# zdebruine/singlet

Measured on AMD Instinct MI355X. Metric: ALS iterations/sec (1M cells x 30k genes, 5% nnz, k=50), higher is better.
Workload: dtype f64

## Files before the change

### singlet_amd/csrc/kernels_tiled.hip

```cpp
#include "sgl_internal.h"
#include <atomic>
#include <hipcub/hipcub.hpp>
#include <stdlib.h>
#include <utility>
#include <type_traits>

#define TILED_NW 8
#define TILED_CW 64
#define TILED_NP 32
#define TILED_LDS_BYTES (160 * 1024 - 512)
#define TILED_SLACK 4096

__device__ __forceinline__ int64_t tiled_slot_col(const int32_t* __restrict__ perm, int64_t ncol, int64_t wb, int h, int p, int nsl) {
    const int64_t pos = wb * (TILED_NP * nsl) + nsl * p + h;
    if (pos >= ncol) return -1;
    return perm ? (int64_t)perm[pos] : pos;
}

__device__ __forceinline__ int tiled_ranges_of(int64_t wb, int R, int64_t tail_wg0, int tail_R) {
    return (tail_R > 1 && tail_wg0 >= 0 && wb / TILED_NW >= tail_wg0) ? tail_R : R;
}
__device__ __forceinline__ int tiled_range_end(int b, int T, int NB, int nr) {
    const int t = b >> 1;
    const int y = (int)(((int64_t)(t + 1) * nr - 1) / T);
    const int b1 = 2 * (int)(((int64_t)(y + 1) * T) / nr);
    return b1 < NB ? b1 : NB;
}

__global__ __launch_bounds__(256) void tiled_count_kernel(const int64_t* __restrict__ seg, const int32_t* __restrict__ perm, int64_t ncol,
                                                          int T, int NB, int64_t nwb, int R, int64_t tail_wg0, int tail_R,
                                                          uint8_t* __restrict__ cnt, uint16_t* __restrict__ ahead,
                                                          int64_t* __restrict__ chunk_entries, int nsl) {
    const int lane = threadIdx.x & 63, p = lane & 31;
    const int64_t wb = ((int64_t)blockIdx.x * blockDim.x + threadIdx.x) >> 6;
    if (wb >= nwb) return;
    const int gps = 16 / nsl;
    int64_t col[4];
    for (int h = 0; h < 4; ++h) col[h] = h < nsl ? tiled_slot_col(perm, ncol, wb, h, p, nsl) : -1;
    const int nr = tiled_ranges_of(wb, R, tail_wg0, tail_R);
    for (int b0 = 0; b0 < NB;) {
        const int b1 = tiled_range_end(b0, T, NB, nr);
        int64_t pos[4];
        for (int h = 0; h < 4; ++h) pos[h] = col[h] >= 0 ? seg[(int64_t)b0 * ncol + col[h]] : 0;
        for (int b = b0; b < b1; ++b) {
            const int hi = b + 2 < b1 ? b + 2 : b1;
            int64_t must = 0, avail = 0, ew[4];
            for (int h = 0; h < 4; ++h) {
                ew[h] = 0;
                if (col[h] >= 0) {
                    const int64_t eb = seg[(int64_t)(b + 1) * ncol + col[h]];
                    ew[h] = seg[(int64_t)hi * ncol + col[h]];
                    must = eb - pos[h] > must ? eb - pos[h] : must;
                    avail = ew[h] - pos[h] > avail ? ew[h] - pos[h] : avail;
                }
            }
            int g = (int)((must + 3) >> 2);
            const int cap = (int)((avail + 3) >> 2) - g;
            int tot = g;
            for (int o = 16; o > 0; o >>= 1) tot += __shfl_xor(tot, o, 32);
            const int rem = (gps - (tot & (gps - 1))) & (gps - 1);
            int suf = cap;
            for (int o = 1; o < 32; o <<= 1) {
                const int v = __shfl_down(suf, o, 32);
                if (p + o < 32) suf += v;
            }
            const int above = suf - cap;
            int extra = rem - above < cap ? rem - above : cap;
            if (extra < 0) extra = 0;
            const int all = __shfl(suf, 0, 32);
            if (p == TILED_NP - 1 && rem > all) extra += rem - all;
            g += extra;
            const int64_t u = wb * NB + b;
            if (lane < 32) {
                cnt[u * TILED_NP + p] = (uint8_t)g;
                for (int h = 0; h < nsl; ++h)
                    ahead[u * (TILED_NP * nsl) + nsl * p + h] = col[h] >= 0 ? (uint16_t)(pos[h] - seg[(int64_t)b * ncol + col[h]]) : (uint16_t)0;
            }
            if (lane == 0) chunk_entries[u] = (int64_t)(tot + rem) * 4 * nsl;
            for (int h = 0; h < 4; ++h) pos[h] += (4 * (int64_t)g < ew[h] - pos[h]) ? 4 * (int64_t)g : ew[h] - pos[h];
        }
        b0 = b1;
    }
}

__global__ __launch_bounds__(256) void tiled_fill_kernel(const double* __restrict__ x, const int32_t* __restrict__ idx,
                                                         const int64_t* __restrict__ seg, const int32_t* __restrict__ perm,
                                                         int64_t ncol, int T, int NB, int64_t nwb, int R, int64_t tail_wg0, int tail_R,
                                                         int D, int row_bytes, const uint8_t* __restrict__ cnt,
                                                         const uint16_t* __restrict__ ahead, const int64_t* __restrict__ cstart,
                                                         uint32_t* __restrict__ sroff, double* __restrict__ sx,
                                                         int masked, uint64_t seed, SglDiv inv_density, int mask_t,
                                                         int64_t col_off, int64_t row_off, int nsl) {
    const int lane = threadIdx.x & 63;
    const int eps = 64 / nsl, eps_sh = nsl == 4 ? 4 : 5;
    const int64_t gw = ((int64_t)blockIdx.x * blockDim.x + threadIdx.x) >> 6;
    const int64_t nw = ((int64_t)gridDim.x * blockDim.x) >> 6;
    for (int64_t u = gw; u < nwb * NB; u += nw) {
        const int64_t wb = u / NB;
        const int b = (int)(u - wb * NB);
        const int b1 = tiled_range_end(b, T, NB, tiled_ranges_of(wb, R, tail_wg0, tail_R));
        const int hi = b + 2 < b1 ? b + 2 : b1;
        const int64_t c0 = cstart[u];
        int P = 0;
        for (int p = 0; p < TILED_NP; ++p) {
            const int n4 = 4 * (int)cnt[u * TILED_NP + p];
            if (n4 == 0) continue;
            for (int h = 0; h < nsl; ++h) {
                const int64_t col = tiled_slot_col(perm, ncol, wb, h, p, nsl);
                int64_t a = 0, e = 0;
                if (col >= 0) {
                    a = seg[(int64_t)b * ncol + col] + ahead[u * (TILED_NP * nsl) + nsl * p + h];
                    e = seg[(int64_t)hi * ncol + col];
                }
                for (int q = lane; q < n4; q += 64) {
                    uint32_t ro = 0;
                    double xv = 0.0;
                    if (a + q < e) {
                        const int32_t r = idx[a + q];
                        const int blk = r >= (b + 1) * D ? b + 1 : b;
                        ro = (uint32_t)((blk & 1) * D + (r - blk * D)) * (uint32_t)row_bytes;
                        xv = x[a + q];
                        if (masked) {
                            const uint64_t gc = (uint64_t)(col + col_off), gr = (uint64_t)(r + row_off);
                            if (mask_t ? sgl_draw(seed, gr, gc, inv_density) : sgl_draw(seed, gc, gr, inv_density)) xv = 0.0;
                        }
                    }
                    const int pos = P + q;
                    const int64_t dst = c0 + (int64_t)(pos >> eps_sh) * 64 + h * eps + (pos & (eps - 1));
                    if (sroff != nullptr) sroff[dst] = ro;
                    sx[dst] = xv;
                }
            }
            P += n4;
        }
    }
}

__global__ __launch_bounds__(256) void tiled_gtab_kernel(const uint8_t* __restrict__ cnt, const int64_t* __restrict__ cstart,
                                                         int64_t nchunks, int nsl, uint16_t* __restrict__ gtab) {
    const int lane = threadIdx.x & 63;
    const int64_t gw = ((int64_t)blockIdx.x * blockDim.x + threadIdx.x) >> 6;
    const int64_t nw = ((int64_t)gridDim.x * blockDim.x) >> 6;
    for (int64_t u = gw; u < nchunks; u += nw) {
        int64_t g0 = cstart[u] / (4 * nsl);
        for (int p = 0; p < TILED_NP; ++p) {
            const int n = (int)cnt[u * TILED_NP + p];
            for (int q = lane; q < n; q += 64) gtab[g0 + q] = (uint16_t)(0x8000u | (unsigned)(4 * p));
            g0 += n;
        }
    }
}

template <typename T_>
static int t_alloc(T_** p, size_t count) {
    *p = nullptr;
    if (count == 0) count = 1;
    hipError_t e = sgl_pool_malloc((void**)p, count * sizeof(T_));
    if (e != hipSuccess) {
        (void)hipGetLastError();
        sgl_set_error("hipMalloc of %zu bytes failed: %s", count * sizeof(T_), hipGetErrorString(e));
        return SGL_ENOMEM;
    }
    return SGL_OK;
}

template <typename T_>
static int t_reserve(T_** p, size_t* cap, size_t count) {
    if (*p != nullptr && *cap >= count) return SGL_OK;
    if (*p) (void)sgl_pool_free(*p);
    *p = nullptr;
    *cap = 0;
    const size_t want = count + count / 32 + 64;
    SGLCHK(t_alloc(p, want));
    *cap = want;
    return SGL_OK;
}

void sgl_tiled_free(DevTiled& S) {
    if (S.seg) (void)sgl_pool_free(S.seg);
    if (S.perm) (void)sgl_pool_free(S.perm);
    if (S.roff) (void)sgl_pool_free(S.roff);
    if (S.x) (void)sgl_pool_free(S.x);
    if (S.cstart) (void)sgl_pool_free(S.cstart);
    if (S.cnt) (void)sgl_pool_free(S.cnt);
    if (S.ahead) (void)sgl_pool_free(S.ahead);
    if (S.gtab) (void)sgl_pool_free(S.gtab);
    if (S.part) (void)sgl_pool_free(S.part);
    if (S.xm) (void)sgl_pool_free(S.xm);
    S = DevTiled();
}

static bool tiled_sort_columns() {
    const char* e = getenv("SGL_TILED_SORT");
    return !(e && *e == '0');
}

__global__ void tiled_col_keys_kernel(const int64_t* __restrict__ p, int64_t ncol, uint32_t* __restrict__ keys, int32_t* __restrict__ iota) {
    for (int64_t c = (int64_t)blockIdx.x * blockDim.x + threadIdx.x; c < ncol; c += (int64_t)gridDim.x * blockDim.x) {
        keys[c] = (uint32_t)(p[c + 1] - p[c]);
        iota[c] = (int32_t)c;
    }
}

static int tiled_build_perm(sgl_ctx* c, const DevCSC& M, DevTiled& S) {
    hipStream_t s = c->stream;
    const int64_t n = M.ncol;
    SGLCHK(t_reserve(&S.perm, &S.cap_perm, (size_t)n));
    uint32_t *keys = nullptr, *keys_out = nullptr;
    int32_t* iota = nullptr;
    void* tmp = nullptr;
    int rc = t_alloc(&keys, (size_t)n);
    if (rc == SGL_OK) rc = t_alloc(&keys_out, (size_t)n);
    if (rc == SGL_OK) rc = t_alloc(&iota, (size_t)n);
    if (rc == SGL_OK && n > 0) {
        const int64_t blocks = std::min<int64_t>((n + 255) / 256, 4096);
        tiled_col_keys_kernel<<<dim3((unsigned)blocks), dim3(256), 0, s>>>(M.p, n, keys, iota);
        size_t tmp_bytes = 0;
        if (hipcub::DeviceRadixSort::SortPairsDescending(nullptr, tmp_bytes, keys, keys_out, iota, S.perm, n, 0, 32, s) != hipSuccess) rc = SGL_EHIP;
        if (rc == SGL_OK && sgl_pool_malloc(&tmp, tmp_bytes ? tmp_bytes : 1) != hipSuccess) { (void)hipGetLastError(); rc = SGL_ENOMEM; }
        if (rc == SGL_OK && hipcub::DeviceRadixSort::SortPairsDescending(tmp, tmp_bytes, keys, keys_out, iota, S.perm, n, 0, 32, s) != hipSuccess) rc = SGL_EHIP;
    }
    static_assert(TILED_CW == 64, "pair layout: 64 columns per wave");
    std::vector<uint32_t> top_v((size_t)TILED_NW * TILED_CW * 2);
    uint32_t* top = top_v.data();
    const int64_t ntop = std::min<int64_t>(n, (int64_t)top_v.size());
    if (rc == SGL_OK && ntop > 0 && hipMemcpyAsync(top, keys_out, sizeof(uint32_t) * (size_t)ntop, hipMemcpyDeviceToHost, s) != hipSuccess) rc = SGL_EHIP;
    const hipError_t e = hipStreamSynchronize(s);
    if (rc == SGL_OK && e == hipSuccess) {
        int64_t tn = 0, tn2 = 0;
        for (int64_t q = 0; q < ntop; ++q) {
            if (q < TILED_NW * TILED_CW) tn += top[q];
            tn2 += top[q];
        }
        S.top_share = M.nnz > 0 ? (double)tn / (double)M.nnz : 0.0;
        S.top_share4 = M.nnz > 0 ? (double)tn2 / (double)M.nnz : 0.0;
    }
    if (keys) (void)sgl_pool_free(keys);
    if (keys_out) (void)sgl_pool_free(keys_out);
    if (iota) (void)sgl_pool_free(iota);
    if (tmp) (void)sgl_pool_free(tmp);
    if (rc == SGL_OK && e != hipSuccess) rc = SGL_EHIP;
    if (rc != SGL_OK) { sgl_set_error("tiled build: sorting the columns by their non-zero count failed"); return rc; }
    S.perm_nnz = M.nnz;
    return SGL_OK;
}

void sgl_trace_setup(const char* what);

int sgl_tiled_build(sgl_ctx* c, const DevCSC& M, int k, DevTiled& S) {
    hipStream_t s = c->stream;
    const int nsl = (k <= 32 && !getenv("SGL_TILED_NO_QUAD")) ? 4 : 2;
    if (S.built && S.k == k && S.NSL == nsl && S.ncol == M.ncol && S.nrow == M.nrow && S.src_nnz == M.nnz && (S.perm != nullptr) == tiled_sort_columns())
        return SGL_OK;
    S.built = false;
    S.xm_mask_t = -1;
    S.k = k;
    S.NSL = nsl;
    S.CW = TILED_NP * nsl;
    const int KS = nsl == 4 ? 32 : ((k + 1) & ~1);
    S.KS = KS;
    int TR = TILED_LDS_BYTES / (KS * 8);
    TR = TR / 8 * 8;
    if (TR > 984) TR = 984;
    if (TR < 8 || k > 64) { sgl_set_error("tiled accumulate: k=%d unsupported", k); return SGL_EINVAL; }
    S.nwb = ((int64_t)M.ncol + S.CW - 1) / S.CW;
    {
        const int64_t groups = (S.nwb + TILED_NW - 1) / TILED_NW, T0 = ((int64_t)M.nrow + TR - 1) / TR;
        if (groups * T0 < 256 && !getenv("SGL_TILED_FULL_TILES")) {
            const int64_t want = std::min<int64_t>((256 + groups - 1) / groups, ((int64_t)M.nrow + 127) / 128);
            if (want > T0) TR = std::min<int>(TR, (int)(((((int64_t)M.nrow + want - 1) / want) + 7) / 8 * 8));
        }
    }
    S.TR = TR;
    S.T = (int)((M.nrow + TR - 1) / TR);
    const int D = TR / 2;
    S.NB = (int)((M.nrow + D - 1) / D);
    S.ncol = M.ncol;
    S.nrow = M.nrow;
    S.src_nnz = M.nnz;
    const int64_t nchunks = S.nwb * S.NB;

    int rc = SGL_OK;
    if (!tiled_sort_columns()) {
        if (S.perm) { (void)sgl_pool_free(S.perm); S.perm = nullptr; S.cap_perm = 0; }
    } else if (!S.perm || S.perm_nnz != M.nnz || S.cap_perm < (size_t)M.ncol) {
        rc = tiled_build_perm(c, M, S);
    }
    sgl_trace_setup("  stream: column order");
    const double E_est = (double)M.nnz * 1.06;
    const int64_t nwg_x = (S.nwb + TILED_NW - 1) / TILED_NW;
    int R = 1;
    const int r_fill = nwg_x < 1024 ? (int)std::max<int64_t>(1, (512 + nwg_x - 1) / nwg_x) : 1;
    const double top_share = nsl == 4 ? S.top_share4 : S.top_share;
    const bool skewed = S.perm && top_share * (double)nwg_x > 1.5;
    const int r_bal = skewed ? (int)std::min<double>(256.0, ceil(top_share * 256.0 / 0.35)) : 1;
    if (r_bal > r_fill) {
        double best = -1.0;
        const int rmin = std::max(r_fill, (int)std::min<int64_t>(r_bal, std::max(1, S.T)));
        if (rmin > S.T) R = std::max(1, S.T);
        for (int r = rmin; r <= std::min<int64_t>(S.T, rmin + rmin / 4 + 4); ++r) {
            const int tpr = (S.T + r - 1) / r;
            const int reff = (S.T + tpr - 1) / tpr;
            const double wgs = (double)nwg_x * reff;
            const double eff = wgs / (ceil(wgs / 256.0) * 256.0);
            if (eff > best + 1e-9) { best = eff; R = reff; }
        }
    } else if (r_fill > 1 && S.T > 1) {
        const double t_tile = E_est / (double)nsl / ((double)nwg_x * (double)S.T) * 2.4e-9 + 2.5e-6;
        const double t_wg = 6e-6;
        double best = 1e300;
        for (int r = 1; r <= std::min<int64_t>(S.T, 64); ++r) {
            const double wgs = (double)nwg_x * r;
            const double rounds = ceil(wgs / 256.0);
            const int largest = (S.T + r - 1) / r;
            const double cost = rounds * ((double)largest * t_tile + t_wg) + (r > 1 ? (double)r * (double)k * (double)M.ncol * 16.0 / 4e12 : 0.0);
            if (cost < best * (1.0 - 1e-9)) { best = cost; R = r; }
        }
    }
    if (const char* fr = getenv("SGL_TILED_RANGES")) {
        if (atoi(fr) > 0) R = atoi(fr);
    }
    S.range_fastest = r_bal > r_fill;
    S.R = std::max(1, std::min(R, std::max(1, S.T)));
    S.tiles_per_range = (S.T + S.R - 1) / S.R;
    S.tail_wg0 = -1;
    S.tail_R = 1;
    if (S.R == 1 && !S.range_fastest && nwg_x > 256 && S.T > 1 && E_est >= (double)(4ll << 20) && !getenv("SGL_TILED_NO_TAIL")) {
        const int64_t tail = nwg_x % 256;
        if (tail > 0) {
            const double t_tile = E_est / (double)nsl / ((double)nwg_x * (double)S.T) * 2.4e-9 + 2.5e-6;
            const double t_wg = 6e-6;
            const double tail_cols = (double)tail * TILED_NW * S.CW;
            double best = (double)S.T * t_tile + t_wg;
            int Rt = 1;
            for (int r = 2; r <= std::min<int64_t>(S.T, 16); ++r) {
                const double rounds = ceil((double)tail * r / 256.0);
                const double cost = rounds * ((double)((S.T + r - 1) / r) * t_tile + t_wg) + (double)r * (double)k * tail_cols * 16.0 / 4e12;
                if (cost < best * (1.0 - 1e-9)) { best = cost; Rt = r; }
            }
            if (Rt > 1) { S.tail_wg0 = nwg_x - tail; S.tail_R = Rt; }
        }
    }
    if (rc == SGL_OK) rc = t_reserve(&S.seg, &S.cap_seg, (size_t)(S.NB + 1) * (size_t)M.ncol);
    sgl_trace_setup("  stream: segment buffer reserved");
    DevCSC tmp = M;
    tmp.tile_rows = D;
    tmp.ntiles = S.NB;
    tmp.seg = S.seg;
    if (rc == SGL_OK) rc = k_build_segments(s, tmp);
    int64_t* chunk_entries = nullptr;
    if (rc == SGL_OK) rc = t_alloc(&chunk_entries, (size_t)nchunks);
    if (rc == SGL_OK) rc = t_reserve(&S.cnt, &S.cap_cnt, (size_t)nchunks * TILED_NP);
    if (rc == SGL_OK) rc = t_reserve(&S.ahead, &S.cap_ahead, (size_t)nchunks * (size_t)S.CW);
    if (rc == SGL_OK) rc = t_reserve(&S.cstart, &S.cap_cstart, (size_t)nchunks + 1);
    if (rc == SGL_OK && S.nwb > 0) {
        tiled_count_kernel<<<dim3((unsigned)((S.nwb + 3) / 4)), dim3(256), 0, s>>>(S.seg, S.perm, M.ncol, S.T, S.NB, S.nwb, S.R,
                                                                                   S.tail_wg0, S.tail_R, S.cnt, S.ahead, chunk_entries, nsl);
        if (hipGetLastError() != hipSuccess) { sgl_set_error("tiled build: count kernel launch failed"); rc = SGL_EHIP; }
    }
    if (rc == SGL_OK) rc = k_exclusive_scan(c, chunk_entries, S.cstart, nchunks);
    if (rc == SGL_OK) rc = k_scan_total(s, chunk_entries, S.cstart, nchunks);
    int64_t E = 0;
    if (rc == SGL_OK) {
        if (hipMemcpyAsync(&E, S.cstart + nchunks, sizeof(int64_t), hipMemcpyDeviceToHost, s) != hipSuccess ||
            hipStreamSynchronize(s) != hipSuccess) { sgl_set_error("tiled build: reading the stream size failed"); rc = SGL_EHIP; }
    }
    S.E = E;
    sgl_trace_setup("  stream: segments, counts, scan");
    if (rc == SGL_OK) rc = t_reserve(&S.roff, &S.cap_roff, (size_t)E + TILED_SLACK);
    if (rc == SGL_OK) rc = t_reserve(&S.x, &S.cap_x, (size_t)E + TILED_SLACK);
    sgl_trace_setup("  stream: roff / x buffers reserved");
    if (rc == SGL_OK) {
        if (hipMemsetAsync(S.roff + E, 0, TILED_SLACK * sizeof(uint32_t), s) != hipSuccess ||
            hipMemsetAsync(S.x + E, 0, TILED_SLACK * sizeof(double), s) != hipSuccess) { sgl_set_error("tiled build: clearing the stream slack failed"); rc = SGL_EHIP; }
    }
    if (rc == SGL_OK && nchunks > 0) {
        int64_t blocks = (nchunks + 3) / 4;
        if (blocks > 256 * 64) blocks = 256 * 64;
        tiled_fill_kernel<<<dim3((unsigned)blocks), dim3(256), 0, s>>>(M.x, M.i, S.seg, S.perm, M.ncol, S.T, S.NB, S.nwb, S.R, S.tail_wg0,
                                                                       S.tail_R, D, KS * 8, S.cnt, S.ahead, S.cstart, S.roff, S.x,
                                                                       0, 0, sgl_div_make(1), 0, 0, 0, nsl);
        if (hipGetLastError() != hipSuccess) { sgl_set_error("tiled build: fill kernel launch failed"); rc = SGL_EHIP; }
    }
    const size_t ngroups = (size_t)(E / (4 * nsl));
    if (rc == SGL_OK) rc = t_reserve(&S.gtab, &S.cap_gtab, ngroups + 256);
    if (rc == SGL_OK) {
        if (hipMemsetAsync(S.gtab + ngroups, 0, 256 * sizeof(uint16_t), s) != hipSuccess) { sgl_set_error("tiled build: clearing the schedule slack failed"); rc = SGL_EHIP; }
    }
    if (rc == SGL_OK && nchunks > 0) {
        int64_t blocks = (nchunks + 3) / 4;
        if (blocks > 256 * 64) blocks = 256 * 64;
        tiled_gtab_kernel<<<dim3((unsigned)blocks), dim3(256), 0, s>>>(S.cnt, S.cstart, nchunks, nsl, S.gtab);
        if (hipGetLastError() != hipSuccess) { sgl_set_error("tiled build: schedule kernel launch failed"); rc = SGL_EHIP; }
    }
    if (rc == SGL_OK && S.R > 1) rc = t_reserve(&S.part, &S.cap_part, (size_t)S.R * (size_t)k * (size_t)M.ncol);
    if (rc == SGL_OK && S.tail_R > 1)
        rc = t_reserve(&S.part, &S.cap_part, (size_t)S.tail_R * (size_t)k * (size_t)((nwg_x - S.tail_wg0) * TILED_NW * S.CW));
    hipError_t e = hipStreamSynchronize(s);
    if (chunk_entries) (void)sgl_pool_free(chunk_entries);
    if (rc == SGL_OK && e != hipSuccess) { sgl_set_error("tiled build failed: %s", hipGetErrorString(e)); rc = SGL_EHIP; }
    if (rc != SGL_OK) { sgl_tiled_free(S); return rc; }
    S.built = true;
    ++S.builds;
    return rc;
}

int sgl_tiled_mask_values(sgl_ctx* c, const DevCSC& M, DevTiled& S, uint64_t seed, uint64_t inv_density, int mask_t,
                          int64_t col_off, int64_t row_off) {
    if (!S.built || !S.seg || !S.ahead) { sgl_set_error("masked values: no entry stream"); return SGL_ESTATE; }
    if (S.xm && S.xm_seed == seed && S.xm_inv == inv_density && S.xm_mask_t == mask_t) return SGL_OK;
    hipStream_t s = c->stream;
    S.xm_mask_t = -1;
    SGLCHK(t_reserve(&S.xm, &S.cap_xm, (size_t)S.E + TILED_SLACK));
    HIPCHK(hipMemsetAsync(S.xm + S.E, 0, TILED_SLACK * sizeof(double), s));
    const int64_t nchunks = S.nwb * S.NB;
    if (nchunks > 0) {
        const int KS = S.KS;
        int64_t blocks = (nchunks + 3) / 4;
        if (blocks > 256 * 64) blocks = 256 * 64;
        tiled_fill_kernel<<<dim3((unsigned)blocks), dim3(256), 0, s>>>(M.x, M.i, S.seg, S.perm, M.ncol, S.T, S.NB, S.nwb, S.R, S.tail_wg0,
                                                                       S.tail_R, S.TR / 2, KS * 8, S.cnt, S.ahead, S.cstart, nullptr, S.xm,
                                                                       1, seed, sgl_div_make(inv_density), mask_t, col_off, row_off, S.NSL);
        HIPCHK(hipGetLastError());
    }
    S.xm_seed = seed; S.xm_inv = inv_density; S.xm_mask_t = mask_t;
    return SGL_OK;
}


__device__ __forceinline__ void acc_load(int idx4, double& v0, double& v1) {
    int a, b, c, d;
    asm volatile(
        "s_set_gpr_idx_on %4, gpr_idx(SRC0)\n\tv_mov_b32 %0, v128\n\tv_mov_b32 %1, v129\n\tv_mov_b32 %2, v130\n\t"
        "v_mov_b32 %3, v131\n\ts_set_gpr_idx_off"
        : "=v"(a), "=v"(b), "=v"(c), "=v"(d) : "s"(idx4) : "memory");
    v0 = __hiloint2double(b, a);
    v1 = __hiloint2double(d, c);
}

#include "acc_tiled_gen.inc"

template <int NSL>
__device__ __forceinline__ void tiled_stage(double* __restrict__ tile, const double* __restrict__ src, int rows, int k, int KS, int ldf,
                                            bool sync) {
    const int n = rows * k;
    if constexpr (NSL == 4) {
        const int c16 = (int)threadIdx.x & 15, r0 = (int)threadIdx.x >> 4;
        constexpr int RPR = 64 * TILED_NW / 16;
        const bool vec = ((k | ldf) & 1) == 0 && (reinterpret_cast<uintptr_t>(src) & 15) == 0;
        if (vec) {
            constexpr int RST = 4;
            double2 stg[RST];
            const bool cact = 2 * c16 < k;
#pragma unroll
            for (int j = 0; j < RST; ++j) {
                const int r = r0 + j * RPR;
                stg[j] = double2{0.0, 0.0};
                if (cact && r < rows) stg[j] = *reinterpret_cast<const double2*>(src + (int64_t)r * ldf + 2 * c16);
            }
            if (sync) __syncthreads();
            for (int rb = 0; rb < rows; rb += RST * RPR) {
#pragma unroll
                for (int j = 0; j < RST; ++j) {
                    const int r = rb + r0 + j * RPR;
                    if (cact && r < rows) *reinterpret_cast<double2*>(tile + r * 32 + 2 * c16) = stg[j];
                }
                if (rb + RST * RPR < rows) {
#pragma unroll
                    for (int j = 0; j < RST; ++j) {
                        const int r = rb + RST * RPR + r0 + j * RPR;
                        stg[j] = double2{0.0, 0.0};
                        if (cact && r < rows) stg[j] = *reinterpret_cast<const double2*>(src + (int64_t)r * ldf + 2 * c16);
                    }
                }
            }
        } else {
            if (sync) __syncthreads();
            for (int r = r0; r < rows; r += RPR) {
                if (c16 < k) tile[r * 32 + c16] = src[(int64_t)r * ldf + c16];
                if (c16 + 16 < k) tile[r * 32 + c16 + 16] = src[(int64_t)r * ldf + c16 + 16];
            }
        }
    } else {
        if (sync) __syncthreads();
        if (((k | ldf) & 1) == 0 && (reinterpret_cast<uintptr_t>(src) & 15) == 0) {
            const int hp = k >> 1;
            for (int e = (int)threadIdx.x; e < rows * hp; e += 64 * TILED_NW) {
                const int r = e / hp, c2 = (e - r * hp) * 2;
                *reinterpret_cast<double2*>(tile + r * KS + c2) = *reinterpret_cast<const double2*>(src + (int64_t)r * ldf + c2);
            }
        } else {
            for (int e = (int)threadIdx.x; e < n; e += 64 * TILED_NW) {
                const int r = e / k, f = e - r * k;
                tile[r * KS + f] = src[(int64_t)r * ldf + f];
            }
        }
        if (KS != k)
            for (int r = (int)threadIdx.x; r < rows; r += 64 * TILED_NW) tile[r * KS + k] = 0.0;
    }
}

#define TILED_PIECES 10
static_assert(TILED_PIECES * 64 * TILED_NW * 16 >= TILED_LDS_BYTES / 2, "the pieces must cover a whole ring slot");
#define TILED_PIECE_CLOBBERS "v24", "v25", "v26", "v27", "v28", "v29", "v30", "v31", "v32", "v33", "v34", "v35", "v36", "v37", "v38", \
    "v39", "v40", "v41", "v42", "v43", "v44", "v45", "v46", "v47", "v48", "v49", "v50", "v51", "v52", "v53", "v54", "v55", "v56", "v57", \
    "v58", "v59", "v60", "v61", "v62", "v63"

#define TILED_ISSUE_PIECE(regs, off) \
    "v_add_u32 %[t], " off ", %[o]\n\tv_min_u32 %[t], %[last], %[t]\n\tglobal_load_dwordx4 " regs ", %[t], %[src]\n\t"

__device__ __forceinline__ void tiled_issue(const double* src, int n) {
    static_assert(TILED_PIECES == 10, "tiled_issue / tiled_commit move ten pieces");
    const unsigned o = threadIdx.x * 16u, last = (unsigned)n * 8u - 16u;
    unsigned t;
    asm volatile(
        "v_min_u32 %[t], %[last], %[o]\n\tglobal_load_dwordx4 v[24:27], %[t], %[src]\n\t"
        TILED_ISSUE_PIECE("v[28:31]", "0x2000") TILED_ISSUE_PIECE("v[32:35]", "0x4000") TILED_ISSUE_PIECE("v[36:39]", "0x6000")
        TILED_ISSUE_PIECE("v[40:43]", "0x8000") TILED_ISSUE_PIECE("v[44:47]", "0xa000") TILED_ISSUE_PIECE("v[48:51]", "0xc000")
        TILED_ISSUE_PIECE("v[52:55]", "0xe000") TILED_ISSUE_PIECE("v[56:59]", "0x10000") TILED_ISSUE_PIECE("v[60:63]", "0x12000")
        : [t] "=&v"(t)
        : [o] "v"(o), [last] "s"(last), [src] "s"(src)
        : TILED_PIECE_CLOBBERS);
}

#define TILED_COMMIT_PIECE(regs, addr, off) \
    "v_cmp_gt_i32 vcc, %[lim], %[a]\n\ts_and_b64 exec, exec, vcc\n\tds_write_b128 " addr ", " regs off "\n\ts_sub_i32 %[lim], %[lim], 0x2000\n\t"
#define TILED_COMMIT_ASM(wait) \
    "s_waitcnt vmcnt(" wait ")\n\ts_mov_b64 %[sv], exec\n\t" \
    TILED_COMMIT_PIECE("v[24:27]", "%[a]", "") TILED_COMMIT_PIECE("v[28:31]", "%[a]", " offset:8192") \
    TILED_COMMIT_PIECE("v[32:35]", "%[a]", " offset:16384") TILED_COMMIT_PIECE("v[36:39]", "%[a]", " offset:24576") \
    TILED_COMMIT_PIECE("v[40:43]", "%[a]", " offset:32768") TILED_COMMIT_PIECE("v[44:47]", "%[a]", " offset:40960") \
    TILED_COMMIT_PIECE("v[48:51]", "%[a]", " offset:49152") TILED_COMMIT_PIECE("v[52:55]", "%[a]", " offset:57344") \
    TILED_COMMIT_PIECE("v[56:59]", "%[a1]", "") TILED_COMMIT_PIECE("v[60:63]", "%[a1]", " offset:8192") \
    "s_mov_b64 exec, %[sv]\n\ts_waitcnt lgkmcnt(0)"
#define TILED_COMMIT_OPERANDS : [sv] "=&s"(sv), [lim] "+s"(lim) : [a] "v"(a), [a1] "v"(a + 65536u) : "vcc", "scc", "memory"

__device__ __forceinline__ void tiled_commit(double* tile, int n, bool ring_after) {
    typedef __attribute__((address_space(3))) char lds_char;
    const unsigned base = (unsigned)(uintptr_t)(lds_char*)tile;
    const unsigned a = base + threadIdx.x * 16u;
    int lim = (int)(base + (unsigned)n * 8u);
    uint64_t sv;
    if (ring_after)
        asm volatile(TILED_COMMIT_ASM("16") TILED_COMMIT_OPERANDS);
    else
        asm volatile(TILED_COMMIT_ASM("0") TILED_COMMIT_OPERANDS);
}

#define ACC_TILED_PARAMS                                                                                                          \
    const uint32_t* __restrict__ sroff, const double* __restrict__ sx, const int64_t* __restrict__ cstart,                            \
        const uint8_t* __restrict__ cnt, int T, int NB, int64_t nwb, const double* __restrict__ F, int k, int TR, int64_t nrow,       \
        int tiles_per_range, double* __restrict__ Bout, int64_t ncol, int KS, int ldf, int ldb, int64_t slab,                        \
        const int32_t* __restrict__ perm, int range_fastest, const uint16_t* __restrict__ gtab, int tail_wg0, int tail_R,            \
        double* __restrict__ tail_part, int64_t tail_slab
#define ACC_TILED_ARGS \
    sroff, sx, cstart, cnt, T, NB, nwb, F, k, TR, nrow, tiles_per_range, Bout, ncol, KS, ldf, ldb, slab, perm, range_fastest, gtab, \
        tail_wg0, tail_R, tail_part, tail_slab
template <int NSL>
__device__ __forceinline__ void acc_tiled_body(ACC_TILED_PARAMS) {
    asm volatile("" ::: "v255");
    extern __shared__ __attribute__((aligned(16))) char smem[];
    double* tile = reinterpret_cast<double*>(smem);
    const int lane = threadIdx.x & 63;
    const int wave = __builtin_amdgcn_readfirstlane((int)(threadIdx.x >> 6));
    unsigned bx = blockIdx.x, by = blockIdx.y;
    if (range_fastest) {
        const unsigned unit = blockIdx.x + gridDim.x * blockIdx.y, nranges = gridDim.y;
        bx = unit / nranges;
        by = unit - bx * nranges;
    }
    unsigned nry = gridDim.y;
    bool tail_piece = false;
    if (tail_R > 1 && (int)bx >= tail_wg0) {
        const unsigned u = bx - (unsigned)tail_wg0;
        bx = (unsigned)tail_wg0 + u / (unsigned)tail_R;
        by = u % (unsigned)tail_R;
        nry = (unsigned)tail_R;
        tail_piece = true;
    }
    const int64_t wb = (int64_t)bx * TILED_NW + wave;
    const int t0 = (int)(((int64_t)by * T) / nry);
    const int t1 = (int)((((int64_t)by + 1) * T) / nry);
    const int D = TR >> 1;
    const int b0 = 2 * t0, b1 = 2 * t1 < NB ? 2 * t1 : NB;
    const bool wact = wb < nwb;
    typedef __attribute__((address_space(3))) char lds_char;
    constexpr int LMASK = NSL == 4 ? 15 : 31;
    const unsigned lane16 = (unsigned)(uintptr_t)(lds_char*)smem + (lane & LMASK) * 16;
    const unsigned slot = NSL == 2 ? (unsigned)((lane >> 5) * 32 + (lane & 15)) : (unsigned)lane;
    const unsigned voff4 = slot * 4, voff8 = slot * 8;
    constexpr unsigned LAP_R = (NSL == 4 ? 256u : 128u) * 8u;
    const unsigned pfl = (unsigned)lane * (LAP_R / 64u) + (unsigned)ACC_TILED_PF_LAPS * LAP_R;

    asm volatile(ACC_TILED_ZERO_ASM ::: "memory");

    uint64_t rp = 0, xp = 0;
    int phase = 0;
    int64_t pos_next = 0;
    if (wact) {
        const int64_t pos = cstart[wb * NB + b0];
        pos_next = cstart[wb * NB + b0 + 1];
        const uint64_t r_ = reinterpret_cast<uint64_t>(sroff + pos), x_ = reinterpret_cast<uint64_t>(sx + pos);
        rp = ((uint64_t)(uint32_t)__builtin_amdgcn_readfirstlane((unsigned)(r_ >> 32)) << 32) | (uint32_t)__builtin_amdgcn_readfirstlane((unsigned)r_);
        xp = ((uint64_t)(uint32_t)__builtin_amdgcn_readfirstlane((unsigned)(x_ >> 32)) << 32) | (uint32_t)__builtin_amdgcn_readfirstlane((unsigned)x_);
        if constexpr (NSL == 4)
            asm volatile(ACC_TILED4_RING_FILL_ASM : [rp] "+s"(rp), [xp] "+s"(xp) : [voff4] "v"(voff4), [voff8] "v"(voff8) : ACC_TILED_CLOBBERS);
        else
            asm volatile(ACC_TILED2_RING_FILL_ASM : [rp] "+s"(rp), [xp] "+s"(xp) : [voff4] "v"(voff4), [voff8] "v"(voff8) : ACC_TILED_CLOBBERS);
    }
    if constexpr (NSL == 4) {
        for (int e = (int)threadIdx.x; e < TILED_LDS_BYTES / 8; e += 64 * TILED_NW) tile[e] = 0.0;
    }

    const bool pf = NSL == 2 && KS == k && ldf == k;
    auto block_rows = [&](int j) { const int64_t row0 = (int64_t)j * D; return (int)(nrow - row0 < D ? nrow - row0 : D); };
    int64_t pos_cur = wact ? cstart[wb * NB + b0] : 0;
    for (int b = b0; b < b1; ++b) {
        const int nsets = (int)((pos_next - pos_cur) >> 6);
        const int64_t pos_chunk = pos_cur;
        pos_cur = pos_next;
        if (wact && b + 1 < b1) pos_next = cstart[wb * NB + b + 2];

        if (pf) {
            if (b == b0) {
#pragma clang loop unroll(disable)
                for (int j = b; j <= b + 1 && j < b1; ++j) {
                    tiled_issue(F + (int64_t)j * D * ldf, block_rows(j) * k);
                    tiled_commit(tile + (j & 1) * D * KS, block_rows(j) * k, false);
                }
                __syncthreads();
            }
            if (b + 2 < b1) tiled_issue(F + (int64_t)(b + 2) * D * ldf, block_rows(b + 2) * k);
        } else {
#pragma clang loop unroll(disable)
            for (int j = b == b0 ? b : b + 1; j <= b + 1 && j < b1; ++j) {
                const int64_t row0 = (int64_t)j * D;
                tiled_stage<NSL>(tile + (j & 1) * D * KS, F + row0 * ldf, block_rows(j), k, KS, ldf, j == b || b != b0);
            }
            if (b == b0 || b + 1 < b1) {
                __builtin_amdgcn_s_waitcnt(0x0F70);
                __syncthreads();
            }
        }
        if (wact && nsets > 0) {
            const uint64_t t_ = reinterpret_cast<uint64_t>(gtab + pos_chunk / (4 * NSL));
            const uint64_t tp = ((uint64_t)(uint32_t)__builtin_amdgcn_readfirstlane((unsigned)(t_ >> 32)) << 32) | (uint32_t)__builtin_amdgcn_readfirstlane((unsigned)t_);
            if constexpr (NSL == 2)
                asm volatile(ACC_TILED2_CHUNK_ASM
                             : [rp] "+s"(rp), [xp] "+s"(xp), [phase] "+s"(phase)
                             : [ns] "s"(2 * nsets), [tp] "s"(tp), [lane16] "v"(lane16), [voff4] "v"(voff4), [voff8] "v"(voff8), [pfl] "v"(pfl)
                             : ACC_TILED_CHUNK_CLOBBERS);
            else
                asm volatile(ACC_TILED4_CHUNK_ASM
                             : [rp] "+s"(rp), [xp] "+s"(xp), [phase] "+s"(phase)
                             : [ns] "s"(nsets), [tp] "s"(tp), [lane16] "v"(lane16), [voff4] "v"(voff4), [voff8] "v"(voff8), [pfl] "v"(pfl)
                             : ACC_TILED_CHUNK_CLOBBERS);
        }
        if (pf && b + 2 < b1) {
            __syncthreads();
            tiled_commit(tile + (b & 1) * D * KS, block_rows(b + 2) * k, wact && nsets >= 4);
            __syncthreads();
        }
    }
    asm volatile("s_waitcnt vmcnt(0)" ::: "memory");
    if (wact) {
        double* out = Bout + (size_t)by * (size_t)slab;
        const int f = 2 * (lane & LMASK);
        const int64_t tail_pos0 = (int64_t)tail_wg0 * TILED_NW * (TILED_NP * NSL);
        for (int p = 0; p < TILED_NP; ++p) {
            double v0, v1;
            acc_load(4 * p, v0, v1);
            const int h = NSL == 4 ? (lane >> 4) : (lane >> 5);
            const int64_t col = tiled_slot_col(perm, ncol, wb, h, p, NSL);
            if (col >= 0) {
                if (tail_piece) {
                    const int64_t pos = wb * (TILED_NP * NSL) + NSL * p + h;
                    double* o = tail_part + (size_t)by * (size_t)tail_slab + (pos - tail_pos0) * k;
                    if (f < k) o[f] = v0;
                    if (f + 1 < k) o[f + 1] = v1;
                } else {
                    if (f < k) out[col * ldb + f] = v0;
                    if (f + 1 < k) out[col * ldb + f + 1] = v1;
                }
            }
        }
    }
}

template <int NSL>
__global__ __launch_bounds__(512) __attribute__((amdgpu_waves_per_eu(8, 8))) void acc_tiled_kernel(ACC_TILED_PARAMS) {
    acc_tiled_body<NSL>(ACC_TILED_ARGS);
}
template <>
__global__ __launch_bounds__(512) __attribute__((amdgpu_waves_per_eu(8, 8), amdgpu_num_vgpr(12))) void acc_tiled_kernel<2>(ACC_TILED_PARAMS) {
    acc_tiled_body<2>(ACC_TILED_ARGS);
}

__global__ void acc_tiled_reduce_kernel(const double* __restrict__ part, int R, int64_t n, int k, int ldb, double* __restrict__ B) {
    for (int64_t e = (int64_t)blockIdx.x * blockDim.x + threadIdx.x; e < n; e += (int64_t)gridDim.x * blockDim.x) {
        double s = part[e];
        for (int r = 1; r < R; ++r) s += part[(size_t)r * n + e];
        if (ldb == k) {
            B[e] = s;
        } else {
            const int64_t col = e / k;
            B[col * ldb + (e - col * k)] = s;
        }
    }
}

__global__ void acc_tiled_reduce_tail_kernel(const double* __restrict__ part, int R, int64_t slab, int64_t pos0, int64_t ncol,
                                             const int32_t* __restrict__ perm, int k, int ldb, double* __restrict__ B) {
    const int64_t n = (ncol - pos0) * k;
    for (int64_t e = (int64_t)blockIdx.x * blockDim.x + threadIdx.x; e < n; e += (int64_t)gridDim.x * blockDim.x) {
        double s = part[e];
        for (int r = 1; r < R; ++r) s += part[(size_t)r * slab + e];
        const int64_t q = e / k;
        const int64_t col = perm ? (int64_t)perm[pos0 + q] : pos0 + q;
        B[col * ldb + (e - q * k)] = s;
    }
}

int k_acc_tiled(hipStream_t s, const DevTiled& S, const double* F, int ldf, double* B, int ldb, int kf, const double* xvals) {
    if (S.ncol <= 0) return SGL_OK;
    if (kf <= 0 || kf > S.k) { sgl_set_error("k_acc_tiled: bad part size %d (stream built for %d)", kf, S.k); return SGL_EINVAL; }
    const int KS = S.KS;
    const size_t lds = S.NSL == 4 ? (size_t)TILED_LDS_BYTES + 512 : (size_t)S.TR * KS * 8 + 512;
    static std::atomic<bool> attr_set[64];
    int dev = 0;
    HIPCHK(hipGetDevice(&dev));
    if (dev < 0 || dev >= 64 || !attr_set[dev]) {
        HIPCHK(hipFuncSetAttribute(reinterpret_cast<const void*>(&acc_tiled_kernel<2>),
                                   hipFuncAttributeMaxDynamicSharedMemorySize, TILED_LDS_BYTES + 512));
        HIPCHK(hipFuncSetAttribute(reinterpret_cast<const void*>(&acc_tiled_kernel<4>),
                                   hipFuncAttributeMaxDynamicSharedMemorySize, TILED_LDS_BYTES + 512));
        if (dev >= 0 && dev < 64) attr_set[dev] = true;
    }
    const int64_t nwg_x = (S.nwb + TILED_NW - 1) / TILED_NW;
    const bool slabs = S.R > 1;
    double* out = slabs ? S.part : B;
    const int64_t n = (int64_t)kf * S.ncol;
    const bool tail = !slabs && S.tail_R > 1 && S.tail_wg0 >= 0;
    const int64_t tail_cols = tail ? (nwg_x - S.tail_wg0) * TILED_NW * S.CW : 0;
    const int64_t tail_slab = tail_cols * kf;
    const dim3 grid(tail ? (unsigned)(S.tail_wg0 + (nwg_x - S.tail_wg0) * S.tail_R) : (unsigned)nwg_x, (unsigned)S.R);
    auto launch = [&](auto nsl) {
        acc_tiled_kernel<decltype(nsl)::value><<<grid, dim3(64 * TILED_NW), lds, s>>>(
            S.roff, xvals ? xvals : S.x, S.cstart, S.cnt, S.T, S.NB, S.nwb, F, kf, S.TR, S.nrow, S.tiles_per_range, out, S.ncol, KS, ldf,
            slabs ? kf : ldb, slabs ? n : 0, S.perm, S.range_fastest ? 1 : 0, S.gtab, tail ? (int)S.tail_wg0 : -1, tail ? S.tail_R : 1,
            S.part, tail_slab);
    };
    if (S.NSL == 4) launch(std::integral_constant<int, 4>());
    else launch(std::integral_constant<int, 2>());
    HIPCHK(hipGetLastError());
    if (tail) {
        const int64_t pos0 = S.tail_wg0 * TILED_NW * S.CW;
        const int64_t ne = (S.ncol - pos0) * kf;
        if (ne > 0) {
            int64_t blocks = (ne + 255) / 256;
            if (blocks > 4096) blocks = 4096;
            acc_tiled_reduce_tail_kernel<<<dim3((unsigned)blocks), dim3(256), 0, s>>>(S.part, S.tail_R, tail_slab, pos0, S.ncol, S.perm, kf, ldb, B);
            HIPCHK(hipGetLastError());
        }
    }
    if (slabs) {
        int64_t blocks = (n + 255) / 256;
        if (blocks > 4096) blocks = 4096;
        acc_tiled_reduce_kernel<<<dim3((unsigned)blocks), dim3(256), 0, s>>>(S.part, S.R, n, kf, ldb, B);
        HIPCHK(hipGetLastError());
    }
    return SGL_OK;
}

int k_acc_tiled_all(hipStream_t s, const DevTiled& S, const double* F, double* B, int k, const double* xvals) {
    for (int f0 = 0; f0 < k; f0 += S.k) {
        const int kf = (k - f0 < S.k) ? (k - f0) : S.k;
        SGLCHK(k_acc_tiled(s, S, F + f0, k, B + f0, k, kf, xvals));
    }
    return SGL_OK;
}

int tiled_part_size(int k) {
    if (k <= 64) return k;
    if (k > SGL_MAX_K) return 0;
    const bool quad = !getenv("SGL_TILED_NO_QUAD");
    const int parts = quad ? (k <= 96 ? 3 : (k + 31) / 32) : (k + 63) / 64;
    return ((k + parts - 1) / parts + 1) & ~1;
}
```

Before: 41.66.

## Balance per-chunk group counts across warps in a workgroup during tiled build

The count kernel now launches one workgroup of TILED_NW wavefronts per tile group and shares each wavefront's group total through LDS. Each wavefront pads its per-chunk group count up toward the workgroup maximum, using only entries already available in its columns, before the usual alignment padding. The aim is to equalize stream chunk lengths across the wavefronts that later consume them together in the fill/solve kernels, reducing load imbalance and idle waves. It adds a __syncthreads per chunk in the build and may lengthen the stream slightly.

```diff
diff --git a/singlet_amd/csrc/kernels_tiled.hip b/singlet_amd/csrc/kernels_tiled.hip
--- a/singlet_amd/csrc/kernels_tiled.hip
+++ b/singlet_amd/csrc/kernels_tiled.hip
@@ -27,17 +27,19 @@
     return b1 < NB ? b1 : NB;
 }
 
-__global__ __launch_bounds__(256) void tiled_count_kernel(const int64_t* __restrict__ seg, const int32_t* __restrict__ perm, int64_t ncol,
-                                                          int T, int NB, int64_t nwb, int R, int64_t tail_wg0, int tail_R,
-                                                          uint8_t* __restrict__ cnt, uint16_t* __restrict__ ahead,
-                                                          int64_t* __restrict__ chunk_entries, int nsl) {
-    const int lane = threadIdx.x & 63, p = lane & 31;
-    const int64_t wb = ((int64_t)blockIdx.x * blockDim.x + threadIdx.x) >> 6;
-    if (wb >= nwb) return;
+__global__ __launch_bounds__(64 * TILED_NW) void tiled_count_kernel(const int64_t* __restrict__ seg, const int32_t* __restrict__ perm, int64_t ncol,
+                                                                   int T, int NB, int64_t nwb, int R, int64_t tail_wg0, int tail_R,
+                                                                   uint8_t* __restrict__ cnt, uint16_t* __restrict__ ahead,
+                                                                   int64_t* __restrict__ chunk_entries, int nsl) {
+    __shared__ int wtot[2][TILED_NW];
+    const int lane = threadIdx.x & 63, p = lane & 31, w = (int)(threadIdx.x >> 6);
+    const int64_t wb = (int64_t)blockIdx.x * TILED_NW + w;
+    const bool live = wb < nwb;
     const int gps = 16 / nsl;
     int64_t col[4];
-    for (int h = 0; h < 4; ++h) col[h] = h < nsl ? tiled_slot_col(perm, ncol, wb, h, p, nsl) : -1;
+    for (int h = 0; h < 4; ++h) col[h] = (live && h < nsl) ? tiled_slot_col(perm, ncol, wb, h, p, nsl) : -1;
     const int nr = tiled_ranges_of(wb, R, tail_wg0, tail_R);
+    int buf = 0;
     for (int b0 = 0; b0 < NB;) {
         const int b1 = tiled_range_end(b0, T, NB, nr);
         int64_t pos[4];
@@ -55,9 +57,31 @@
                 }
             }
             int g = (int)((must + 3) >> 2);
-            const int cap = (int)((avail + 3) >> 2) - g;
+            int64_t lmin = INT64_MAX;
+            for (int h = 0; h < nsl; ++h) {
+                const int64_t l = col[h] >= 0 ? ew[h] - pos[h] - 4 * (int64_t)g : 0;
+                lmin = l < lmin ? l : lmin;
+            }
+            const int fcap = lmin > 0 ? (int)(lmin >> 2) : 0;
             int tot = g;
             for (int o = 16; o > 0; o >>= 1) tot += __shfl_xor(tot, o, 32);
+            if (lane == 0) wtot[buf][w] = live ? tot : 0;
+            __syncthreads();
+            int tmax = 0;
+            for (int q = 0; q < TILED_NW; ++q) tmax = wtot[buf][q] > tmax ? wtot[buf][q] : tmax;
+            buf ^= 1;
+            const int need = ((tmax + gps - 1) & ~(gps - 1)) - tot;
+            int fsuf = fcap;
+            for (int o = 1; o < 32; o <<= 1) {
+                const int v = __shfl_down(fsuf, o, 32);
+                if (p + o < 32) fsuf += v;
+            }
+            int fx = need - (fsuf - fcap) < fcap ? need - (fsuf - fcap) : fcap;
+            if (fx < 0) fx = 0;
+            const int ftot = need < __shfl(fsuf, 0, 32) ? need : __shfl(fsuf, 0, 32);
+            g += fx;
+            tot += ftot;
+            const int cap = (int)((avail + 3) >> 2) - g;
             const int rem = (gps - (tot & (gps - 1))) & (gps - 1);
             int suf = cap;
             for (int o = 1; o < 32; o <<= 1) {
@@ -71,12 +95,12 @@
             if (p == TILED_NP - 1 && rem > all) extra += rem - all;
             g += extra;
             const int64_t u = wb * NB + b;
-            if (lane < 32) {
+            if (live && lane < 32) {
                 cnt[u * TILED_NP + p] = (uint8_t)g;
                 for (int h = 0; h < nsl; ++h)
                     ahead[u * (TILED_NP * nsl) + nsl * p + h] = col[h] >= 0 ? (uint16_t)(pos[h] - seg[(int64_t)b * ncol + col[h]]) : (uint16_t)0;
             }
-            if (lane == 0) chunk_entries[u] = (int64_t)(tot + rem) * 4 * nsl;
+            if (live && lane == 0) chunk_entries[u] = (int64_t)(tot + rem) * 4 * nsl;
             for (int h = 0; h < 4; ++h) pos[h] += (4 * (int64_t)g < ew[h] - pos[h]) ? 4 * (int64_t)g : ew[h] - pos[h];
         }
         b0 = b1;
@@ -354,8 +378,8 @@
     if (rc == SGL_OK) rc = t_reserve(&S.ahead, &S.cap_ahead, (size_t)nchunks * (size_t)S.CW);
     if (rc == SGL_OK) rc = t_reserve(&S.cstart, &S.cap_cstart, (size_t)nchunks + 1);
     if (rc == SGL_OK && S.nwb > 0) {
-        tiled_count_kernel<<<dim3((unsigned)((S.nwb + 3) / 4)), dim3(256), 0, s>>>(S.seg, S.perm, M.ncol, S.T, S.NB, S.nwb, S.R,
-                                                                                   S.tail_wg0, S.tail_R, S.cnt, S.ahead, chunk_entries, nsl);
+        tiled_count_kernel<<<dim3((unsigned)nwg_x), dim3(64 * TILED_NW), 0, s>>>(S.seg, S.perm, M.ncol, S.T, S.NB, S.nwb, S.R,
+                                                                                 S.tail_wg0, S.tail_R, S.cnt, S.ahead, chunk_entries, nsl);
         if (hipGetLastError() != hipSuccess) { sgl_set_error("tiled build: count kernel launch failed"); rc = SGL_EHIP; }
     }
     if (rc == SGL_OK) rc = k_exclusive_scan(c, chunk_entries, S.cstart, nchunks);
```

After: 42.05 (median of 6 runs). No clear change (+0.9%).
